# GothiProCoder/OCR-System

Measured on AMD Instinct MI355X. Metric: pages/sec end-to-end det+rec, A4@200DPI, higher is better.
Workload: dtype bf16; 1 GPU; end-to-end det+rec, batch=64 A4@200DPI pages per GPU (BASELINE configs[3]); pages_per_gpu=64, global_batch=64, lines_last_step=3279, pages_gathered_last_step=64, parallelism=pages sharded dp1, 1 all-gather/step, ranks=1, input=pages pre-decoded (uint8 RGB) and resident in HBM when the timed region starts, det_sub_batch=64

## Files before the change

### ocr-system_amd/csrc/mbconv.h

```cpp
#pragma once
#include "common.h"

struct MbParams {
    const bf16_t* x;
    const bf16_t* we;
    const float* be;
    const bf16_t* wd;
    const float* bd;
    bf16_t* d;
    int N, H, W, cin, expc, Ho, act;
    float* pool;
};

constexpr int MB_STRIP = 32;
inline int mb_strips(int W) { return (W + MB_STRIP - 1) / MB_STRIP; }

size_t mbconv_expand_packed_elems(int expc, int cin);
void mbconv_pack_expand(const bf16_t* w, int expc, int cin, bf16_t* out);
size_t mbconv_lds_bytes(const MbParams& p, int k);
bool mbconv_supported(const MbParams& p, int k, int sh);
hipError_t mbconv_launch(const MbParams& p, int k, int sh, hipStream_t st);
hipError_t se_pool_launch(const bf16_t* d, float* pool, int N, int Ho, int W, int C, hipStream_t st);
```

### ocr-system_amd/csrc/mbconv.hip

```cpp
#include "mbconv.h"

namespace {

__device__ __forceinline__ void unpack8(const uint4 v, float* f) {
    f[0] = __uint_as_float(v.x << 16); f[1] = __uint_as_float(v.x & 0xFFFF0000u);
    f[2] = __uint_as_float(v.y << 16); f[3] = __uint_as_float(v.y & 0xFFFF0000u);
    f[4] = __uint_as_float(v.z << 16); f[5] = __uint_as_float(v.z & 0xFFFF0000u);
    f[6] = __uint_as_float(v.w << 16); f[7] = __uint_as_float(v.w & 0xFFFF0000u);
}
__device__ __forceinline__ uint4 pack8(const float* f) {
    return make_uint4(pack_bf16x2(f[0], f[1]), pack_bf16x2(f[2], f[3]), pack_bf16x2(f[4], f[5]), pack_bf16x2(f[6], f[7]));
}

constexpr int MB_TW = 32, MB_KSMAX = 3;

template <int K, int SH, int ACT>
__global__ __launch_bounds__(256, 2) void mbconv_kernel(const MbParams p) {
    constexpr int PAD = K / 2, EW = MB_TW + 2 * PAD, XG = 4;
    extern __shared__ __attribute__((aligned(16))) unsigned char smem[];
    const int tid = threadIdx.x, lane = tid & 63, wave = tid >> 6, r = lane & 31, h = lane >> 5;
    const int expc = p.expc, cg = expc >> 3;
    const int pitch = expc * 2 + 16;
    const int tile_bytes = (p.H * EW * pitch + 15) & ~15;
    float* wl = reinterpret_cast<float*>(smem + tile_bytes);
    for (int i = tid; i < K * K * expc; i += 256) {
        const int tap = i / expc, c = i - tap * expc;
        wl[((tap * 2 + ((c >> 2) & 1)) * cg + (c >> 3)) * 4 + (c & 3)] = bf16_to_f32(p.wd[i]);
    }
    float* bl = wl + K * K * expc;
    for (int i = tid; i < expc; i += 256) bl[i] = p.bd[i];

    const int ksteps = p.cin >> 4;
    const int mtiles = (expc + 31) >> 5;
    const int npix = p.H * EW, ptiles = (npix + 31) >> 5;
    const int strips_x = (p.W + MB_TW - 1) / MB_TW;
    const int nitems = p.N * strips_x;

    for (int item = blockIdx.x; item < nitems; item += gridDim.x) {
        const int n = item / strips_x, x0 = (item - n * strips_x) * MB_TW;
        __syncthreads();
        for (int pt = wave; pt < ptiles; pt += 4) {
            const int pi = pt * 32 + r;
            const bool valid = pi < npix;
            const int row = pi / EW, col = pi - row * EW;
            const int gx = x0 - PAD + col;
            const bool inimg = valid && gx >= 0 && gx < p.W;
            bf16x8_t bfr[MB_KSMAX];
#pragma unroll
            for (int ks = 0; ks < MB_KSMAX; ++ks) {
                uint4 v = make_uint4(0, 0, 0, 0);
                if (ks < ksteps && inimg) v = *reinterpret_cast<const uint4*>(p.x + (((size_t)n * p.H + row) * p.W + gx) * p.cin + ks * 16 + h * 8);
                bfr[ks] = *reinterpret_cast<const bf16x8_t*>(&v);
            }
            unsigned char* trow = smem + (size_t)pi * pitch;
            for (int mt = 0; mt < mtiles; ++mt) {
                f32x16_t acc;
#pragma unroll
                for (int j = 0; j < 16; ++j) acc[j] = 0.f;
#pragma unroll
                for (int ks = 0; ks < MB_KSMAX; ++ks)
                    if (ks < ksteps) {
                        const bf16x8_t afr = *reinterpret_cast<const bf16x8_t*>(p.we + ((((size_t)mt * ksteps + ks) * 2 + h) * 32 + r) * 8);
                        acc = __builtin_amdgcn_mfma_f32_32x32x16_bf16(afr, bfr[ks], acc, 0, 0, 0);
                    }
#pragma unroll
                for (int g = 0; g < 4; ++g) {
                    const int c = mt * 32 + 8 * g + 4 * h;
                    if (!valid || c >= expc) continue;
                    uint2 o = make_uint2(0, 0);
                    if (inimg) {
                        const float4 b4 = *reinterpret_cast<const float4*>(p.be + c);
                        o.x = pack_bf16x2(apply_act(acc[4 * g + 0] + b4.x, ACT), apply_act(acc[4 * g + 1] + b4.y, ACT));
                        o.y = pack_bf16x2(apply_act(acc[4 * g + 2] + b4.z, ACT), apply_act(acc[4 * g + 3] + b4.w, ACT));
                    }
                    *reinterpret_cast<uint2*>(trow + c * 2) = o;
                }
            }
        }
        __syncthreads();
        const int groups = 256 / cg, pg = tid / cg, c8_fixed = tid - pg * cg;
        float psum[8] = {0.f, 0.f, 0.f, 0.f, 0.f, 0.f, 0.f, 0.f};
        for (int t = pg; t < p.Ho * (MB_TW / XG) && pg < groups; t += groups) {
            int c8 = c8_fixed;
            asm volatile("" : "+v"(c8));
            const int xg = t % (MB_TW / XG), oy = t / (MB_TW / XG);
            const int ox0 = xg * XG;
            if (x0 + ox0 >= p.W) continue;
            float a[XG][8];
#pragma unroll
            for (int o = 0; o < XG; ++o)
#pragma unroll
                for (int j = 0; j < 8; ++j) a[o][j] = 0.f;
#pragma unroll
            for (int kh = 0; kh < K; ++kh) {
                const int iy = oy * SH - PAD + kh;
                if (iy < 0 || iy >= p.H) continue;
                float in[K + XG - 1][8];
                const unsigned char* src = smem + (size_t)(iy * EW + ox0) * pitch + c8 * 16;
#pragma unroll
                for (int j = 0; j < K + XG - 1; ++j) unpack8(*reinterpret_cast<const uint4*>(src + j * pitch), in[j]);
#pragma unroll
                for (int kw = 0; kw < K; ++kw) {
                    const float4 g0 = *reinterpret_cast<const float4*>(wl + (((kh * K + kw) * 2 + 0) * cg + c8) * 4);
                    const float4 g1 = *reinterpret_cast<const float4*>(wl + (((kh * K + kw) * 2 + 1) * cg + c8) * 4);
                    const float g[8] = {g0.x, g0.y, g0.z, g0.w, g1.x, g1.y, g1.z, g1.w};
#pragma unroll
                    for (int o = 0; o < XG; ++o)
#pragma unroll
                        for (int j = 0; j < 8; ++j) a[o][j] = __builtin_fmaf(in[o + kw][j], g[j], a[o][j]);
                }
            }
            float bb[8];
#pragma unroll
            for (int j = 0; j < 8; ++j) bb[j] = bl[c8 * 8 + j];
            bf16_t* yrow = p.d + (((size_t)n * p.Ho + oy) * p.W + x0 + ox0) * expc + c8 * 8;
#pragma unroll
            for (int o = 0; o < XG; ++o) {
                if (x0 + ox0 + o >= p.W) break;
#pragma unroll
                for (int j = 0; j < 8; ++j) a[o][j] = apply_act(a[o][j] + bb[j], ACT);
                const uint4 v = pack8(a[o]);
                *reinterpret_cast<uint4*>(yrow + (size_t)o * expc) = v;
                if (p.pool != nullptr) {
                    float f[8];
                    unpack8(v, f);
#pragma unroll
                    for (int j = 0; j < 8; ++j) psum[j] += f[j];
                }
            }
        }
        if (p.pool != nullptr) {
            __syncthreads();
            float* red = reinterpret_cast<float*>(smem);
            if (pg < groups) {
#pragma unroll
                for (int j = 0; j < 8; ++j) red[pg * expc + c8_fixed * 8 + j] = psum[j];
            }
            __syncthreads();
            for (int c = tid; c < expc; c += 256) {
                float s = 0.f;
                for (int g = 0; g < groups; ++g) s += red[g * expc + c];
                p.pool[((size_t)n * strips_x + (x0 / MB_TW)) * expc + c] = s;
            }
        }
    }
}

__global__ __launch_bounds__(256) void se_pool_kernel(const bf16_t* d, float* pool, int N, int Ho, int W, int C) {
    extern __shared__ __attribute__((aligned(16))) unsigned char smem[];
    constexpr int XG = 4;
    const int tid = threadIdx.x, cg = C >> 3, groups = 256 / cg, pg = tid / cg, c8 = tid - pg * cg;
    const int strips_x = (W + MB_TW - 1) / MB_TW;
    const int n = blockIdx.x / strips_x, x0 = (blockIdx.x - n * strips_x) * MB_TW;
    float psum[8] = {0.f, 0.f, 0.f, 0.f, 0.f, 0.f, 0.f, 0.f};
    for (int t = pg; t < Ho * (MB_TW / XG) && pg < groups; t += groups) {
        const int xg = t % (MB_TW / XG), oy = t / (MB_TW / XG);
        const int ox0 = xg * XG;
        if (x0 + ox0 >= W) continue;
        const bf16_t* yrow = d + (((size_t)n * Ho + oy) * W + x0 + ox0) * C + c8 * 8;
#pragma unroll
        for (int o = 0; o < XG; ++o) {
            if (x0 + ox0 + o >= W) break;
            float f[8];
            unpack8(*reinterpret_cast<const uint4*>(yrow + (size_t)o * C), f);
#pragma unroll
            for (int j = 0; j < 8; ++j) psum[j] += f[j];
        }
    }
    float* red = reinterpret_cast<float*>(smem);
    if (pg < groups) {
#pragma unroll
        for (int j = 0; j < 8; ++j) red[pg * C + c8 * 8 + j] = psum[j];
    }
    __syncthreads();
    for (int c = tid; c < C; c += 256) {
        float s = 0.f;
        for (int g = 0; g < groups; ++g) s += red[g * C + c];
        pool[((size_t)n * strips_x + (x0 / MB_TW)) * C + c] = s;
    }
}

}

size_t mbconv_expand_packed_elems(int expc, int cin) { return (size_t)((expc + 31) / 32) * (cin / 16) * 2 * 32 * 8; }

void mbconv_pack_expand(const bf16_t* w , int expc, int cin, bf16_t* out) {
    const int mtiles = (expc + 31) / 32, ksteps = cin / 16;
    for (int mt = 0; mt < mtiles; ++mt)
        for (int ks = 0; ks < ksteps; ++ks)
            for (int hh = 0; hh < 2; ++hh)
                for (int rr = 0; rr < 32; ++rr)
                    for (int j = 0; j < 8; ++j) {
                        const int row = mt * 32 + rr, k = ks * 16 + hh * 8 + j;
                        out[((((size_t)mt * ksteps + ks) * 2 + hh) * 32 + rr) * 8 + j] = row < expc ? w[(size_t)row * cin + k] : (bf16_t)0;
                    }
}

bool mbconv_supported(const MbParams& p, int k, int sh) {
    if (!(k == 3 || k == 5) || !(sh == 1 || sh == 2)) return false;
    if (p.cin % 16 != 0 || p.cin > 16 * MB_KSMAX || p.expc % 16 != 0 || p.expc % 8 != 0) return false;
    if (p.act != ACT_RELU && p.act != ACT_HSWISH) return false;
    return mbconv_lds_bytes(p, k) <= 78 * 1024;
}

size_t mbconv_lds_bytes(const MbParams& p, int k) {
    const int ew = MB_TW + 2 * (k / 2), pitch = p.expc * 2 + 16;
    return (((size_t)p.H * ew * pitch + 15) & ~(size_t)15) + ((size_t)k * k * p.expc + p.expc) * sizeof(float);
}

hipError_t se_pool_launch(const bf16_t* d, float* pool, int N, int Ho, int W, int C, hipStream_t st) {
    if (C % 8 != 0 || C / 8 > 256 || C < 8) return hipErrorInvalidValue;
    const size_t lds = (size_t)(256 / (C / 8)) * C * sizeof(float);
    hipLaunchKernelGGL(se_pool_kernel, dim3(N * mb_strips(W)), dim3(256), lds, st, d, pool, N, Ho, W, C);
    return hipGetLastError();
}

hipError_t mbconv_launch(const MbParams& p, int k, int sh, hipStream_t st) {
    if (!mbconv_supported(p, k, sh)) return hipErrorInvalidValue;
    const size_t lds = mbconv_lds_bytes(p, k);
    const int items = p.N * ((p.W + MB_TW - 1) / MB_TW);
    const int grid = items < 4096 ? items : 4096;
#define MB_LAUNCH(K_, SH_, A_)                                                                                                    \
    {                                                                                                                            \
        auto kern = mbconv_kernel<K_, SH_, A_>;                                                                                  \
        { hipError_t e = locr_dyn_lds(reinterpret_cast<const void*>(kern), 80 * 1024); if (e != hipSuccess) return e; }                                                                                                                        \
        hipLaunchKernelGGL(kern, dim3(grid), dim3(256), lds, st, p);                                                             \
    }
#define MB_ACT(K_, SH_) { if (p.act == ACT_RELU) MB_LAUNCH(K_, SH_, ACT_RELU) else MB_LAUNCH(K_, SH_, ACT_HSWISH) }
    if (k == 3 && sh == 1) MB_ACT(3, 1)
    else if (k == 3 && sh == 2) MB_ACT(3, 2)
    else if (k == 5 && sh == 1) MB_ACT(5, 1)
    else MB_ACT(5, 2)
#undef MB_ACT
#undef MB_LAUNCH
    return hipGetLastError();
}
```

Before: 1528 pages/sec.

## Software-pipeline MBConv expand MFMA units and size grid to resident CUs

New measurement: 1561 pages/sec, median of 6. 1.02x the previous value.

```diff
diff --git a/ocr-system_amd/csrc/mbconv.h b/ocr-system_amd/csrc/mbconv.h
--- a/ocr-system_amd/csrc/mbconv.h
+++ b/ocr-system_amd/csrc/mbconv.h
@@ -15,6 +15,19 @@
 constexpr int MB_STRIP = 32;
 inline int mb_strips(int W) { return (W + MB_STRIP - 1) / MB_STRIP; }
 
+constexpr int MB_WAVES = 4;
+struct MbUnit { int pt, mt; };
+__host__ __device__ inline MbUnit mb_unit_first(int wave, int mtiles) {
+    MbUnit u{0, wave};
+    while (u.mt >= mtiles) { u.mt -= mtiles; ++u.pt; }
+    return u;
+}
+__host__ __device__ inline MbUnit mb_unit_next(MbUnit u, int mtiles) {
+    u.mt += MB_WAVES;
+    while (u.mt >= mtiles) { u.mt -= mtiles; ++u.pt; }
+    return u;
+}
+
 size_t mbconv_expand_packed_elems(int expc, int cin);
 void mbconv_pack_expand(const bf16_t* w, int expc, int cin, bf16_t* out);
 size_t mbconv_lds_bytes(const MbParams& p, int k);
diff --git a/ocr-system_amd/csrc/mbconv.hip b/ocr-system_amd/csrc/mbconv.hip
--- a/ocr-system_amd/csrc/mbconv.hip
+++ b/ocr-system_amd/csrc/mbconv.hip
@@ -1,4 +1,6 @@
 #include "mbconv.h"
+
+#include <algorithm>
 
 namespace {
 
@@ -13,21 +15,101 @@
 }
 
 constexpr int MB_TW = 32, MB_KSMAX = 3;
+constexpr int MB_WGS_PER_CU = 3;
+constexpr size_t MB_LDS_PER_CU = 160 * 1024;
+
+template <int KS>
+struct MbOperands {
+    uint4 a[KS], b[KS];
+    float4 e[4];
+};
+
+template <int EW, int PAD, int KS>
+__device__ __forceinline__ void mb_request(const MbParams& p, const bf16_t* xn, int x0, int r, int h, MbUnit u, MbOperands<KS>& o) {
+    const int pi = u.pt * 32 + r;
+    const int row = pi / EW, col = pi - row * EW;
+    const int gy = min(row, p.H - 1), gx = min(max(x0 - PAD + col, 0), p.W - 1);
+    const bf16_t* xp = xn + (gy * p.W + gx) * p.cin;
+    const bf16_t* wp = p.we + ((u.mt * KS * 2 + h) * 32 + r) * 8;
+#pragma unroll
+    for (int ks = 0; ks < KS; ++ks) {
+        o.a[ks] = *reinterpret_cast<const uint4*>(wp + ks * 512);
+        o.b[ks] = *reinterpret_cast<const uint4*>(xp + ks * 16);
+    }
+#pragma unroll
+    for (int g = 0; g < 4; ++g) o.e[g] = *reinterpret_cast<const float4*>(p.be + u.mt * 32 + 8 * g + 4 * h);
+}
+
+template <int EW, int PAD, int ACT, int KS>
+__device__ __forceinline__ void mb_finish(const MbParams& p, unsigned char* smem, int pitch, int x0, int npix, int r, int h, MbUnit u, const MbOperands<KS>& o) {
+    const int pi = u.pt * 32 + r;
+    const int row = pi / EW, col = pi - row * EW;
+    const int gx = x0 - PAD + col;
+    const bool valid = pi < npix;
+    const unsigned keep = (valid && gx >= 0 && gx < p.W) ? 0xFFFFFFFFu : 0u;
+    f32x16_t acc;
+#pragma unroll
+    for (int j = 0; j < 16; ++j) acc[j] = 0.f;
+#pragma unroll
+    for (int ks = 0; ks < KS; ++ks)
+        acc = __builtin_amdgcn_mfma_f32_32x32x16_bf16(__builtin_bit_cast(bf16x8_t, o.a[ks]), __builtin_bit_cast(bf16x8_t, o.b[ks]), acc, 0, 0, 0);
+    unsigned char* trow = smem + pi * pitch;
+#pragma unroll
+    for (int g = 0; g < 4; ++g) {
+        const int c = u.mt * 32 + 8 * g + 4 * h;
+        const float4 b4 = o.e[g];
+        uint2 v;
+        v.x = pack_bf16x2(apply_act(acc[4 * g + 0] + b4.x, ACT), apply_act(acc[4 * g + 1] + b4.y, ACT)) & keep;
+        v.y = pack_bf16x2(apply_act(acc[4 * g + 2] + b4.z, ACT), apply_act(acc[4 * g + 3] + b4.w, ACT)) & keep;
+        if (valid && c < p.expc) *reinterpret_cast<uint2*>(trow + c * 2) = v;
+    }
+}
+
+template <int EW, int PAD, int ACT, int KS>
+__device__ __forceinline__ void mb_phase1(const MbParams& p, unsigned char* smem, int pitch, int n, int x0, int npix, int ptiles, int mtiles, int wave, int r, int h) {
+    const bf16_t* xn = p.x + (size_t)n * p.H * p.W * p.cin + h * 8;
+    MbUnit u0 = mb_unit_first(wave, mtiles);
+    if (u0.pt >= ptiles) return;
+    MbOperands<KS> o0, o1;
+    mb_request<EW, PAD, KS>(p, xn, x0, r, h, u0, o0);
+    for (;;) {
+        const MbUnit u1 = mb_unit_next(u0, mtiles);
+        if (u1.pt >= ptiles) { mb_finish<EW, PAD, ACT, KS>(p, smem, pitch, x0, npix, r, h, u0, o0); return; }
+        mb_request<EW, PAD, KS>(p, xn, x0, r, h, u1, o1);
+        mb_finish<EW, PAD, ACT, KS>(p, smem, pitch, x0, npix, r, h, u0, o0);
+        u0 = mb_unit_next(u1, mtiles);
+        if (u0.pt >= ptiles) { mb_finish<EW, PAD, ACT, KS>(p, smem, pitch, x0, npix, r, h, u1, o1); return; }
+        mb_request<EW, PAD, KS>(p, xn, x0, r, h, u0, o0);
+        mb_finish<EW, PAD, ACT, KS>(p, smem, pitch, x0, npix, r, h, u1, o1);
+    }
+}
 
 template <int K, int SH, int ACT>
 __global__ __launch_bounds__(256, 2) void mbconv_kernel(const MbParams p) {
     constexpr int PAD = K / 2, EW = MB_TW + 2 * PAD, XG = 4;
     extern __shared__ __attribute__((aligned(16))) unsigned char smem[];
-    const int tid = threadIdx.x, lane = tid & 63, wave = tid >> 6, r = lane & 31, h = lane >> 5;
+    const int tid = threadIdx.x, lane = tid & 63, r = lane & 31, h = lane >> 5;
+    const int wave = __builtin_amdgcn_readfirstlane(tid >> 6);
     const int expc = p.expc, cg = expc >> 3;
     const int pitch = expc * 2 + 16;
     const int tile_bytes = (p.H * EW * pitch + 15) & ~15;
     float* wl = reinterpret_cast<float*>(smem + tile_bytes);
-    for (int i = tid; i < K * K * expc; i += 256) {
-        const int tap = i / expc, c = i - tap * expc;
-        wl[((tap * 2 + ((c >> 2) & 1)) * cg + (c >> 3)) * 4 + (c & 3)] = bf16_to_f32(p.wd[i]);
-    }
     float* bl = wl + K * K * expc;
+    for (int i0 = tid; i0 < K * K * cg; i0 += 4 * 256) {
+        uint4 v[4];
+#pragma unroll
+        for (int j = 0; j < 4; ++j) v[j] = reinterpret_cast<const uint4*>(p.wd)[min(i0 + 256 * j, K * K * cg - 1)];
+#pragma unroll
+        for (int j = 0; j < 4; ++j) {
+            const int i = i0 + 256 * j, tap = i / cg, c8 = i - tap * cg;
+            float f[8];
+            unpack8(v[j], f);
+            if (i < K * K * cg) {
+                *reinterpret_cast<float4*>(wl + ((tap * 2 + 0) * cg + c8) * 4) = make_float4(f[0], f[1], f[2], f[3]);
+                *reinterpret_cast<float4*>(wl + ((tap * 2 + 1) * cg + c8) * 4) = make_float4(f[4], f[5], f[6], f[7]);
+            }
+        }
+    }
     for (int i = tid; i < expc; i += 256) bl[i] = p.bd[i];
 
     const int ksteps = p.cin >> 4;
@@ -39,44 +121,9 @@
     for (int item = blockIdx.x; item < nitems; item += gridDim.x) {
         const int n = item / strips_x, x0 = (item - n * strips_x) * MB_TW;
         __syncthreads();
-        for (int pt = wave; pt < ptiles; pt += 4) {
-            const int pi = pt * 32 + r;
-            const bool valid = pi < npix;
-            const int row = pi / EW, col = pi - row * EW;
-            const int gx = x0 - PAD + col;
-            const bool inimg = valid && gx >= 0 && gx < p.W;
-            bf16x8_t bfr[MB_KSMAX];
-#pragma unroll
-            for (int ks = 0; ks < MB_KSMAX; ++ks) {
-                uint4 v = make_uint4(0, 0, 0, 0);
-                if (ks < ksteps && inimg) v = *reinterpret_cast<const uint4*>(p.x + (((size_t)n * p.H + row) * p.W + gx) * p.cin + ks * 16 + h * 8);
-                bfr[ks] = *reinterpret_cast<const bf16x8_t*>(&v);
-            }
-            unsigned char* trow = smem + (size_t)pi * pitch;
-            for (int mt = 0; mt < mtiles; ++mt) {
-                f32x16_t acc;
-#pragma unroll
-                for (int j = 0; j < 16; ++j) acc[j] = 0.f;
-#pragma unroll
-                for (int ks = 0; ks < MB_KSMAX; ++ks)
-                    if (ks < ksteps) {
-                        const bf16x8_t afr = *reinterpret_cast<const bf16x8_t*>(p.we + ((((size_t)mt * ksteps + ks) * 2 + h) * 32 + r) * 8);
-                        acc = __builtin_amdgcn_mfma_f32_32x32x16_bf16(afr, bfr[ks], acc, 0, 0, 0);
-                    }
-#pragma unroll
-                for (int g = 0; g < 4; ++g) {
-                    const int c = mt * 32 + 8 * g + 4 * h;
-                    if (!valid || c >= expc) continue;
-                    uint2 o = make_uint2(0, 0);
-                    if (inimg) {
-                        const float4 b4 = *reinterpret_cast<const float4*>(p.be + c);
-                        o.x = pack_bf16x2(apply_act(acc[4 * g + 0] + b4.x, ACT), apply_act(acc[4 * g + 1] + b4.y, ACT));
-                        o.y = pack_bf16x2(apply_act(acc[4 * g + 2] + b4.z, ACT), apply_act(acc[4 * g + 3] + b4.w, ACT));
-                    }
-                    *reinterpret_cast<uint2*>(trow + c * 2) = o;
-                }
-            }
-        }
+        if (ksteps == 1) mb_phase1<EW, PAD, ACT, 1>(p, smem, pitch, n, x0, npix, ptiles, mtiles, wave, r, h);
+        else if (ksteps == 2) mb_phase1<EW, PAD, ACT, 2>(p, smem, pitch, n, x0, npix, ptiles, mtiles, wave, r, h);
+        else mb_phase1<EW, PAD, ACT, 3>(p, smem, pitch, n, x0, npix, ptiles, mtiles, wave, r, h);
         __syncthreads();
         const int groups = 256 / cg, pg = tid / cg, c8_fixed = tid - pg * cg;
         float psum[8] = {0.f, 0.f, 0.f, 0.f, 0.f, 0.f, 0.f, 0.f};
@@ -217,9 +264,13 @@
 
 hipError_t mbconv_launch(const MbParams& p, int k, int sh, hipStream_t st) {
     if (!mbconv_supported(p, k, sh)) return hipErrorInvalidValue;
+    if (reinterpret_cast<uintptr_t>(p.wd) & 15) return hipErrorInvalidValue;
     const size_t lds = mbconv_lds_bytes(p, k);
     const int items = p.N * ((p.W + MB_TW - 1) / MB_TW);
-    const int grid = items < 4096 ? items : 4096;
+    int dev = 0, cus = 0;
+    { hipError_t e = hipGetDevice(&dev); if (e == hipSuccess) e = hipDeviceGetAttribute(&cus, hipDeviceAttributeMultiprocessorCount, dev); if (e != hipSuccess) return e; }
+    const int per_cu = (int)std::min<size_t>(MB_WGS_PER_CU, MB_LDS_PER_CU / ((lds + 1023) & ~(size_t)1023));
+    const int grid = std::min(items, cus * per_cu);
 #define MB_LAUNCH(K_, SH_, A_)                                                                                                    \
     {                                                                                                                            \
         auto kern = mbconv_kernel<K_, SH_, A_>;                                                                                  \
```
